# go-compression/raisin

Hardware: AMD Instinct MI355X
Metric: encode+decode MB/s (higher is better)
Workload: dtype u8; 1 GPU; huffman encode+decode, 1024 MiB uniform-random bytes 0x00-0x7F (BASELINE configs[1]), splitmix64 seed 0x5EED0002; algorithm=huffman, bytes_per_gpu=1073741824, chunks=1

## Files before the change

### raisin_amd/csrc/huff_decode.hip

```cpp
#include <chrono>
#include <optional>
#include "codecs.h"
#include "rsn_helpers.h"

namespace rsn {


constexpr int DB = 256;
constexpr int FDB = 256;
constexpr int SW = 8;
constexpr int SBITS = SW * 32;
constexpr int ORG_WORDS = 8;
constexpr int ORG = ORG_WORDS * 32;
constexpr int DATA_WORDS = ORG_WORDS + DB * SW + 8;
constexpr int LUT_BITS_MAX = 11;
constexpr int LUT_WORDS = 1 << LUT_BITS_MAX;
constexpr int OUT_STAGE = DB * 64;
constexpr int OUT_STAGE_RUNE = 40960;
constexpr int CHILD_LDS = 256;
constexpr int LUT2_LDS = 768;
constexpr uint32_t LUT2_GLOBAL_MAX = 1u << 20;
constexpr int SYNC_ROUNDS = 24;
constexpr uint32_t BAD_REL = 0xFFFF;
constexpr uint32_t BAD_POS = 0xFFFFFFFFu;
// ... 219 lines not shown
                }
                const uint32_t er = a.entry_rel[g];
                skip = er == BAD_REL ? e == ~0ull : e == blk_bit0 + er;
            }
            if (__atomic_load_n(a.stuck, __ATOMIC_RELAXED)) skip = 2;
            s_skip = skip;
        }
        __syncthreads();
        if (s_skip == 2) {
            if (live) { a.entry_rel[g] = (uint16_t)BAD_REL; a.exit_rel[g] = (uint16_t)BAD_REL; a.nbyte[g] = 0; }
            if (tid == 0) a.blk_bytes[blk] = 0;
            continue;
        }
        if (s_skip) continue;
        stage_data(a, blk, s_data);
        __syncthreads();

        uint32_t e;
        if (!live) e = BAD_POS;
        else if (g == 0) e = (uint32_t)a.p0 + ORG;
        else if (a.pass == 0 || tid > 0) {
            const long long p0_rel = (long long)a.p0 - (long long)blk_bit0 + ORG;
            if (p0_rel >= (long long)my0) e = (uint32_t)p0_rel;
            else if (a.flat_guess) {
                const unsigned long long d = (unsigned long long)((long long)my0 - p0_rel) + a.min_len - 1;
                e = (uint32_t)(p0_rel + (long long)(d - d % a.min_len));
            } else {
                const uint32_t start = (uint32_t)max(p0_rel, (long long)my0 - a.warm);
                uint32_t q = start;
                (void)advance<ASCII, SHORT, MULTI>(a, s_data, s_lut, lane_r, l2, q, my0, (uint32_t)tid);
                e = q;
            }
        } else {
            const uint32_t xr = a.exit_rel[g - 1];
            e = xr == BAD_REL ? BAD_POS : ORG + xr;
        }
        bool have = false;
        uint32_t x = 0, nb = 0;
        if (live && a.pass > 0 && tid > 0) {
            const uint32_t er = a.entry_rel[g];
            const uint32_t xr = a.exit_rel[g];
            e = er == BAD_REL ? BAD_POS : my0 + er;
            x = xr == BAD_REL ? BAD_POS : lim + xr;
            nb = a.nbyte[g];
            have = true;
        }
        __syncthreads();
        for (int round = 0; round <= DB; round++) {
            if (live && !have) {
                if (e == BAD_POS) { x = BAD_POS; nb = 0; }
                else walk<ASCII, SHORT, MULTI>(a, s_data, s_lut, lane_r, l2, e, lim, (uint32_t)tid + 1u, end_rel, &x, &nb);
                have = true;
            }
            s_exit[tid] = x;
            __syncthreads();
            bool changed = false;
            if (live && tid > 0) {
                const uint32_t en = s_exit[tid - 1];
                if (en != e) { e = en; have = false; changed = true; }
            }
            if (!__syncthreads_or(changed)) break;
            if (round == SYNC_ROUNDS) { if (tid == 0) *a.stuck = 1; break; }
        }
        if (live && !have) { e = BAD_POS; x = BAD_POS; nb = 0; }
        if (live) {
            const uint16_t new_exit = x == BAD_POS ? (uint16_t)BAD_REL : (uint16_t)(x - lim);
            if (a.pass > 0 && tid == DB - 1 && a.exit_rel[g] != new_exit) *a.changed = 1;
            a.entry_rel[g] = e == BAD_POS ? BAD_REL : (uint16_t)(e - my0);
            a.exit_rel[g] = new_exit;
            a.nbyte[g] = (uint16_t)nb;
        }
        unsigned long long sum = live ? nb : 0;
        for (int d = 32; d; d >>= 1) sum += __shfl_down(sum, d);
        if ((tid & 63) == 0) s_part[tid >> 6] = sum;
        __syncthreads();
        if (tid == 0) {
            unsigned long long all = 0;
            for (int k = 0; k < DB / 64; k++) all += s_part[k];
            a.blk_bytes[blk] = all;
        }
    }
}

__global__ __launch_bounds__(256) void k_dec_fix_list(const uint16_t *__restrict__ exit_rel, const uint16_t *__restrict__ entry_rel, uint32_t n_blk,
                                                      uint32_t *__restrict__ list, uint32_t *__restrict__ count) {
    const uint32_t b = blockIdx.x * 256 + threadIdx.x;
    const bool need = b >= 1 && b < n_blk && exit_rel[(size_t)b * DB - 1] != entry_rel[(size_t)b * DB];
    const unsigned long long m = __ballot(need);
    if (!m) return;
    const int lane = threadIdx.x & 63;
    uint32_t base = 0;
    if (lane == 0) base = atomicAdd(count, (uint32_t)__builtin_popcountll(m));
    base = (uint32_t)__builtin_amdgcn_readfirstlane((int)base);
    if (need) list[base + (uint32_t)__builtin_popcountll(m & ((1ull << lane) - 1ull))] = b;
}

constexpr uint32_t PH_CAND = 64;
struct PhaseArgs {
    uint2 *blk_map;
    const uint8_t *true_c;
    uint32_t cand;
};

template <bool ASCII, bool SHORT, bool MULTI>
__global__ __launch_bounds__(DB) void k_dec_phase(DecArgs a, PhaseArgs p, uint32_t n_blk, int mode) {
    __shared__ __attribute__((aligned(1024))) uint32_t s_data[DATA_PHYS];
    __shared__ uint32_t s_lut[LUT_WORDS];
    __shared__ int32_t s_child[SHORT ? 1 : CHILD_LDS];
    __shared__ uint32_t s_lut2[SHORT ? 1 : LUT2_LDS];
    __shared__ uint32_t s_T[64 * PH_CAND];
    const int tid = threadIdx.x;
    const uint32_t lane = tid & 63, wave = tid >> 6;
    const uint32_t lane_r = tid & ((1u << a.rep_log2) - 1);
    stage_lut(a, s_lut);
    if (!SHORT && a.child_n <= (uint32_t)CHILD_LDS) { for (uint32_t i = tid; i < a.child_n; i += DB) s_child[i] = a.child[i]; a.child = s_child; }
    const Lut2 l2{s_lut2, a.lut2_n <= (uint32_t)LUT2_LDS};
    if (!SHORT && l2.in_lds) for (uint32_t i = tid; i < a.lut2_n; i += DB) s_lut2[i] = a.lut2[i];
    for (uint32_t blk = blockIdx.x; blk < n_blk; blk += gridDim.x) {
        const unsigned long long blk_bit0 = (unsigned long long)blk * DB * SBITS;
        const uint32_t L = min((uint32_t)DB, a.n_sub - blk * DB);
        const uint32_t end_rel = (uint32_t)min(a.end - blk_bit0 + ORG, (unsigned long long)(ORG + DB * SBITS + 4096));
        const uint32_t C = p.cand;
        __syncthreads();
        stage_data(a, blk, s_data);
        uint32_t e = mode == 0 ? (uint32_t)tid : (uint32_t)p.true_c[blk];
        if (mode == 2 && e == 0xFF) e = BAD_REL;
        if (blk == 0 && mode == 0 && tid > 0) e = 0x10000u;
        uint32_t bytes = 0;
        const bool follower = mode == 0 ? (uint32_t)tid < C : tid == 0;
        for (uint32_t grp0 = 0; grp0 < L; grp0 += 64) {
            __syncthreads();
            const uint32_t t = grp0 + lane;
            if (t < L) {
                const uint32_t t0 = ORG + t * SBITS, lim = min(t0 + (uint32_t)SBITS, end_rel);
                const uint32_t first = blk == 0 && t == 0 ? (uint32_t)a.p0 : 0u;
                for (uint32_t c0 = wave; c0 < C; c0 += DB / 64) {
                    uint32_t x = BAD_POS, nbs = 0;
                    walk<ASCII, SHORT, MULTI>(a, s_data, s_lut, lane_r, l2, t0 + first + c0, lim, t + 1u, end_rel, &x, &nbs);
                    s_T[lane * PH_CAND + c0] = (x == BAD_POS ? (uint32_t)BAD_REL : x - lim) | nbs << 16;
                }
            }
            __syncthreads();
            if (follower) {
                const uint32_t n_here = min(64u, L - grp0);
                for (uint32_t k = 0; k < n_here; k++) {
                    const uint32_t g = blk * DB + grp0 + k;
                    uint32_t x = BAD_REL, nbs = 0;
                    if (e < C) { const uint32_t v = s_T[k * PH_CAND + e]; x = v & 0xFFFFu; nbs = v >> 16; }
                    else if (e != BAD_REL) e = 0x10000u;
                    if (mode == 2) {
                        a.entry_rel[g] = (uint16_t)(e == BAD_REL || e >= C ? (uint32_t)BAD_REL : (blk == 0 && grp0 + k == 0 ? (uint32_t)a.p0 : e));
                        a.exit_rel[g] = (uint16_t)x; a.nbyte[g] = (uint16_t)nbs;
                    }
                    bytes += nbs;
                    if (e < C || e == BAD_REL) e = x;
                }
            }
        }
        if (follower) {
            if (mode == 0) p.blk_map[(size_t)blk * PH_CAND + tid] = make_uint2(e & 0xFFFFu, e > 0xFFFFu ? 0xFFFFFFFFu : bytes);
            else a.blk_bytes[blk] = bytes;
        }
    }
}

struct Sink {
    uint8_t *wordp; unsigned long long acc; uint32_t cnt, lo;
    __device__ __forceinline__ void start(uint8_t *p) { lo = (uint32_t)((uintptr_t)p & 7); wordp = p - lo; cnt = lo; acc = 0; }
    __device__ __forceinline__ void put(uint32_t b) {
        acc |= (unsigned long long)b << (8 * cnt);
        if (++cnt == 8) {
            if (lo == 0) *reinterpret_cast<unsigned long long *>(wordp) = acc;
            else for (uint32_t k = lo; k < 8; k++) wordp[k] = (uint8_t)(acc >> (8 * k));
            wordp += 8; acc = 0; cnt = 0; lo = 0;
        }
    }
    __device__ __forceinline__ void finish() { for (uint32_t k = lo; k < cnt; k++) wordp[k] = (uint8_t)(acc >> (8 * k)); }
};

template <class Put>
__device__ __forceinline__ void put_rune(uint32_t rune, Put put) {
    if (rune < 0x80) put(rune);
    else if (rune < 0x800) { put(0xC0 | (rune >> 6)); put(0x80 | (rune & 0x3F)); }
    else if (rune < 0x10000) { put(0xE0 | (rune >> 12)); put(0x80 | ((rune >> 6) & 0x3F)); put(0x80 | (rune & 0x3F)); }
    else { put(0xF0 | (rune >> 18)); put(0x80 | ((rune >> 12) & 0x3F)); put(0x80 | ((rune >> 6) & 0x3F)); put(0x80 | (rune & 0x3F)); }
}

template <bool ASCII, bool SHORT, class Put>
__device__ __forceinline__ void emit_walk(const DecArgs &a, const uint32_t *s_data, const uint32_t *s_lut,
                                          uint32_t lane_r, const Lut2 &l2, uint32_t pos, uint32_t lim, Put put) {
    while (pos < lim) {
        const uint32_t r = decode_one<ASCII, SHORT>(a, s_data, s_lut, lane_r, pos, l2);
        if (ASCII) put(r); else put_rune(r, put);
    }
}

#define RSN_EMIT_WORD(p, v) atomicOr((p), (v))
template <bool ASCII, bool SHORT, bool MULTI>
__global__ __launch_bounds__(DB) void k_dec_emit(DecArgs a, uint32_t n_blk) {
    __shared__ __attribute__((aligned(1024))) uint32_t s_data[DATA_PHYS];
    __shared__ uint32_t s_lut[LUT_WORDS];
    constexpr int STAGE = ASCII ? OUT_STAGE : OUT_STAGE_RUNE;
    __shared__ __attribute__((aligned(16))) uint8_t s_out[STAGE + 32];
    __shared__ uint32_t s_wsum[DB / 64];
    __shared__ int32_t s_child[SHORT ? 1 : CHILD_LDS];
    __shared__ uint32_t s_lut2[SHORT ? 1 : LUT2_LDS];
    const int tid = threadIdx.x, lane = tid & 63, wv = tid >> 6;
    const uint32_t lane_r = tid & ((1u << a.rep_log2) - 1);
    const uint32_t my0 = ORG + tid * SBITS;
    stage_lut(a, s_lut);
    if (!SHORT && a.child_n <= (uint32_t)CHILD_LDS) { for (uint32_t i = tid; i < a.child_n; i += DB) s_child[i] = a.child[i]; a.child = s_child; }
    const Lut2 l2{s_lut2, a.lut2_n <= (uint32_t)LUT2_LDS};
    if (!SHORT && l2.in_lds) for (uint32_t i = tid; i < a.lut2_n; i += DB) s_lut2[i] = a.lut2[i];
    if (ASCII) for (int i = tid; i < (STAGE + 32) / 16; i += DB) reinterpret_cast<uint4 *>(s_out)[i] = make_uint4(0, 0, 0, 0);
    for (uint32_t blk = blockIdx.x; blk < n_blk; blk += gridDim.x) {
        const unsigned long long blk_bit0 = (unsigned long long)blk * DB * SBITS;
        const uint32_t g = blk * DB + tid;
        const bool live = g < a.n_sub;
        const uint32_t end_rel = (uint32_t)min(a.end - blk_bit0 + ORG, (unsigned long long)(ORG + DB * SBITS + 4096));
        const uint32_t lim = min(my0 + SBITS, end_rel);
        __syncthreads();
        stage_data(a, blk, s_data);
        const uint32_t nb = live ? a.nbyte[g] : 0;
        const uint32_t er = live ? a.entry_rel[g] : BAD_REL;
        uint32_t incl = nb;
        for (int d = 1; d < 64; d <<= 1) { const uint32_t y = __shfl_up(incl, d); if (lane >= d) incl += y; }
        if (lane == 63) s_wsum[wv] = incl;
        __syncthreads();
        uint32_t wpre = 0, total = 0;
        for (int k = 0; k < DB / 64; k++) { if (k < wv) wpre += s_wsum[k]; total += s_wsum[k]; }
        const uint32_t my_off = wpre + incl - nb;
        if (a.blk_off[blk] + total > a.out_cap) continue;
        uint8_t *dst = a.out + a.blk_off[blk];
        const uint32_t al = (uint32_t)((uintptr_t)dst & 15);
        const bool staged = total + al <= (uint32_t)STAGE;
        if (ASCII && staged) {
            if (live && er != BAD_REL && nb != 0) {
                const uint32_t o0 = al + my_off;
                uint32_t *o = reinterpret_cast<uint32_t *>(s_out) + (o0 >> 2);
                const uint32_t spo = 32u * ((uint32_t)tid + 1u);
                uint32_t cnt = o0 & 3, remaining = nb, pos = my0 + er + spo;
                unsigned long long acc = 0;
                while (remaining) {
                    const uint32_t win = window32_sp(s_data, pos);
                    const uint32_t e = lut_at(a, s_lut, win, lane_r);
                    uint32_t bytes = u_bytes(e);
                    uint32_t take = min(u_n(e), remaining);
                    uint32_t used = u_used(e);
                    if (!SHORT && __ballot((e & 0x80000000u) != 0)) {
                        if (e & 0x80000000u) { uint32_t q = pos - spo; bytes = decode_long(a, s_data, win, e, q, l2); take = 1; used = q + spo - pos; }
                    }
                    acc |= (unsigned long long)bytes << (8 * cnt);
                    cnt += take; remaining -= take; pos += used;
                    if (cnt >= 4) { RSN_EMIT_WORD(o, (uint32_t)acc); o++; acc >>= 32; cnt -= 4; }
                    if (used <= (uint32_t)LUT_BITS_MAX && remaining) {
                        uint32_t e2 = lut_at(a, s_lut, win >> used, lane_r);
                        if (!SHORT) e2 = (int32_t)e2 < 0 ? 0u : e2;
                        {
                            const uint32_t b2 = u_bytes(e2);
                            const uint32_t t2 = min(u_n(e2), remaining);
                            acc |= (unsigned long long)b2 << (8 * cnt);
                            cnt += t2; remaining -= t2; pos += u_used(e2);
                            if (cnt >= 4) { RSN_EMIT_WORD(o, (uint32_t)acc); o++; acc >>= 32; cnt -= 4; }
                        }
                    }
                }
                if (cnt) atomicOr(o, (uint32_t)acc & (0xFFFFFFFFu >> (32 - 8 * cnt)));
            }
        } else if (live && er != BAD_REL && nb != 0) {
            if (staged) {
                uint8_t *o = s_out + al + my_off;
                uint32_t pos = my0 + er;
                emit_walk<ASCII, SHORT>(a, s_data, s_lut, lane_r, l2, pos, lim, [&](uint32_t b) { *o++ = (uint8_t)b; });
            } else {
                Sink sink;
                sink.start(dst + my_off);
                emit_walk<ASCII, SHORT>(a, s_data, s_lut, lane_r, l2, my0 + er, lim, [&](uint32_t b) { sink.put(b); });
                sink.finish();
            }
        }
        if (!staged) continue;
        __syncthreads();
        const uint32_t span = al + total;
        uint8_t *gbase = dst - al;
        for (uint32_t u = tid; u * 16 < span; u += DB) {
            const uint32_t b0 = u * 16;
            if (b0 >= al && b0 + 16 <= span) *reinterpret_cast<uint4 *>(gbase + b0) = *reinterpret_cast<const uint4 *>(s_out + b0);
            else for (uint32_t k = max(b0, al); k < min(b0 + 16, span); k++) gbase[k] = s_out[k];
            if (ASCII) *reinterpret_cast<uint4 *>(s_out + b0) = make_uint4(0, 0, 0, 0);
        }
    }
}

struct FlatArgs {
    const uint8_t *base; size_t nbytes;
    unsigned long long p0;
    unsigned long long n_sym;
    uint8_t *out;
    uint8_t lut[128];
};
constexpr int FLAT_LANE_SYMS = 32;
constexpr int FLAT_SYMS = FDB * FLAT_LANE_SYMS;

template <int L>
__global__ __launch_bounds__(FDB) void k_dec_flat(FlatArgs a) {
    constexpr int WORDS = FDB * L + 2;
    constexpr int RL = 5;
    __shared__ uint32_t s_data[WORDS + WORDS / 32 + 2];
    __shared__ uint32_t s_lut[(1 << L) << RL];
    const int tid = threadIdx.x;
    {
        const uint8_t *lut = (const uint8_t *)__builtin_amdgcn_kernarg_segment_ptr() + offsetof(FlatArgs, lut);
        for (int i = tid; i < ((1 << L) << RL); i += FDB) s_lut[i] = lut[i >> RL];
    }
    const uint32_t n_chunks = (uint32_t)((a.n_sym + FLAT_SYMS - 1) / FLAT_SYMS);
    for (uint32_t chunk = blockIdx.x; chunk < n_chunks; chunk += gridDim.x) {
    const unsigned long long sym0 = (unsigned long long)chunk * FLAT_SYMS;
    const unsigned long long bit0 = a.p0 + sym0 * L;
    const size_t w0 = (size_t)(bit0 >> 5);
    const uint32_t o0 = (uint32_t)(bit0 & 31);
    if ((w0 + WORDS) * 4 <= a.nbytes) {
        const uint32_t *src = reinterpret_cast<const uint32_t *>(a.base) + w0;
        constexpr int PER = (WORDS + FDB - 1) / FDB;
        uint32_t v[PER];
#pragma unroll
        for (int k = 0; k < PER; k++) { const int i = tid + k * FDB; if (i < WORDS) v[k] = ld4<(RSN_NT_MASK & 8) != 0>(src + i); }
#pragma unroll
        for (int k = 0; k < PER; k++) { const int i = tid + k * FDB; if (i < WORDS) s_data[swz(i)] = __builtin_bswap32(v[k]); }
    } else {
        for (int i = tid; i < WORDS; i += FDB) {
            const size_t off = (w0 + i) * 4;
            uint32_t v = 0;
            if (off + 4 <= a.nbytes) v = __builtin_bswap32(*reinterpret_cast<const uint32_t *>(a.base + off));
            else for (int k = 0; k < 4; k++) if (off + k < a.nbytes) v |= (uint32_t)a.base[off + k] << (24 - 8 * k);
            s_data[swz(i)] = v;
        }
    }
    __syncthreads();
    const unsigned long long s_first = sym0 + (unsigned long long)tid * FLAT_LANE_SYMS;
    if (s_first < a.n_sym) {
    const uint32_t lane_r = tid & ((1u << RL) - 1);
    uint32_t w[L + 1], v[L];
#pragma unroll
    for (int j = 0; j <= L; j++) w[j] = s_data[swz(tid * L + j)];
#pragma unroll
    for (int j = 0; j < L; j++) v[j] = (uint32_t)((((unsigned long long)w[j] << 32) | w[j + 1]) >> (32 - o0));
    uint32_t o[8];
#pragma unroll
    for (int k = 0; k < FLAT_LANE_SYMS; k++) {
        constexpr uint32_t mask = (1u << L) - 1;
        const int bp = k * L, wi = bp >> 5, sh = bp & 31;
        uint32_t f;
        if (sh + L <= 32) f = (v[wi] >> (32 - sh - L)) & mask;
        else f = (uint32_t)((((unsigned long long)v[wi] << 32) | v[wi + 1 < L ? wi + 1 : wi]) >> (64 - sh - L)) & mask;
        const uint32_t sym = s_lut[(f << RL) | lane_r];
        if ((k & 3) == 0) o[k >> 2] = sym; else o[k >> 2] |= sym << (8 * (k & 3));
    }
    uint8_t *dst = a.out + s_first;
    if (s_first + FLAT_LANE_SYMS <= a.n_sym) {
        st16<(RSN_NT_MASK & 16) != 0>(reinterpret_cast<uint4 *>(dst), make_uint4(o[0], o[1], o[2], o[3]));
        st16<(RSN_NT_MASK & 16) != 0>(reinterpret_cast<uint4 *>(dst + 16), make_uint4(o[4], o[5], o[6], o[7]));
    } else {
        const uint32_t cnt = (uint32_t)(a.n_sym - s_first);
        for (uint32_t k = 0; k < cnt; k++) dst[k] = (uint8_t)(o[k >> 2] >> (8 * (k & 3)));
    }
    }
    __syncthreads();
    }
}

namespace {

void build_tables(const HuffTree &t, int K, std::vector<uint32_t> &lut, std::vector<int32_t> &child) {
    const uint32_t A = t.n_leaves;
    const size_t n_int = t.freq.size() - A;
    child.assign(2 * std::max<size_t>(n_int, 1), 0);
    for (size_t i = 0; i < n_int; i++) {
        const int32_t id = (int32_t)(A + i);
        const int32_t kids[2] = {t.left[id], t.right[id]};
        for (int b = 0; b < 2; b++)
            child[2 * i + b] = t.is_leaf(kids[b]) ? -(int32_t)(t.rune[kids[b]] + 1) : kids[b] - (int32_t)A;
    }
    lut.assign((size_t)1 << K, 0);
    struct It { int32_t node; uint32_t prefix; int depth; };
    std::vector<It> st;
    st.push_back({t.root, 0, 0});
    while (!st.empty()) {
        const It it = st.back();
        st.pop_back();
        if (t.is_leaf(it.node)) {
            const uint32_t ent = ((uint32_t)it.depth << 24) | t.rune[it.node];
            const uint32_t lo = it.prefix << (K - it.depth);
            for (uint32_t x = 0; x < (1u << (K - it.depth)); x++) lut[lo + x] = ent;
        } else if (it.depth == K) {
            lut[it.prefix] = 0x80000000u | (uint32_t)(it.node - (int32_t)A);
        } else {
            st.push_back({t.right[it.node], (it.prefix << 1) | 1, it.depth + 1});
            st.push_back({t.left[it.node], it.prefix << 1, it.depth + 1});
        }
    }
}

void build_second_level(const std::vector<int32_t> &child, int K, bool byte_alphabet, std::vector<uint32_t> &lut, std::vector<uint32_t> &lut2) {
    lut2.clear();
    const size_t n_int = child.size() / 2;
    std::vector<uint8_t> depth(n_int, 0);
    for (size_t i = 0; i < n_int; i++) {
        unsigned d = 0;
        for (int b = 0; b < 2; b++) { const int32_t k = child[2 * i + b]; d = std::max(d, k < 0 ? 1u : 1u + depth[(size_t)k]); }
        depth[i] = (uint8_t)std::min(d, 255u);
    }
    std::vector<uint32_t> longs;
    for (uint32_t v = 0; v < (1u << K); v++) if (lut[v] & 0x80000000u) longs.push_back(v);
    if (longs.empty()) return;
    auto total = [&](unsigned cap) { uint64_t t = 0; for (uint32_t v : longs) t += 1ull << std::min<unsigned>(depth[lut[v] & 0x3FFFFFFu], cap); return t; };
    unsigned cap = 32u - (unsigned)K;
    if (total(cap) > (uint64_t)LUT2_LDS) {
        const uint64_t budget = byte_alphabet ? (uint64_t)LUT2_LDS : (uint64_t)LUT2_GLOBAL_MAX;
        while (cap > 0 && total(cap) > budget) cap--;
    }
    if (cap == 0) return;
    struct It { int32_t node; uint32_t path; unsigned q; };
    std::vector<It> st;
    for (uint32_t v : longs) {
        const int32_t top = (int32_t)(lut[v] & 0x3FFFFFFu);
        const unsigned sb = std::min<unsigned>(depth[(size_t)top], cap);
        const uint32_t off = (uint32_t)lut2.size();
        lut2.resize(lut2.size() + ((size_t)1 << sb));
        st.push_back({top, 0, 0});
        while (!st.empty()) {
            const It it = st.back();
            st.pop_back();
            if (it.q == sb) { lut2[off + it.path] = 0x80000000u | (uint32_t)it.node; continue; }
            for (int b = 0; b < 2; b++) {
                const int32_t k = child[2 * (size_t)it.node + b];
                const uint32_t path = it.path | ((uint32_t)b << it.q);
                const unsigned q1 = it.q + 1;
                if (k >= 0) { st.push_back({k, path, q1}); continue; }
                const uint32_t ent = ((uint32_t)(K + q1) << 24) | (uint32_t)(-(k + 1));
                for (uint32_t y = 0; y < (1u << (sb - q1)); y++) lut2[off + path + (y << q1)] = ent;
            }
        }
        lut[v] = 0x80000000u | (sb << 26) | off;
    }
}

int rep_for(int K) {
    int r = 0;
    while (r < 5 && ((1 << K) << (r + 1)) <= LUT_WORDS) r++;
    return r;
}

}

int huff_decode_dev(Ctx &c, hipStream_t s, const uint8_t *d_in, size_t n, uint8_t *d_out, size_t out_cap, size_t *out_n, const SliceStream *st) {
    if (((uintptr_t)d_in & 15) || ((uintptr_t)d_out & 15)) return c.fail(RSN_ERR_ARG, "huffman: device buffers must be 16-byte aligned");
    *out_n = 0;
    std::vector<uint8_t> head;
    size_t sep = (size_t)-1;
    for (size_t want = 4096;; want *= 8) {
        const size_t k = std::min(want, n);
        const size_t old = head.size();
        if (k > old) {
            if (st && !st->need_in(k)) return c.fail(RSN_ERR_DEVICE, "huffman: the upload of a sliced call failed");
            void *hpin; int prc = pinned_buf(c, k - old + 64, &hpin); if (prc) return prc;
            RSN_HIP(copy_async(hpin, d_in + old, k - old, hipMemcpyDeviceToHost, s));
            RSN_HIP(hipStreamSynchronize(s));
            head.resize(k);
            memcpy(head.data() + old, hpin, k - old);
        }
        for (size_t i = old ? old - 1 : 0; i + 1 < k; i++) if (head[i] == 0x5C && head[i + 1] == 0x0A) { sep = i; break; }
        if (sep != (size_t)-1 || k == n) break;
    }
    if (sep == (size_t)-1) return c.fail(RSN_ERR_FORMAT, "huffman: no '\\\\\\n' separator (reference: index out of range, huffman.go:264)");
    if (sep + 3 > head.size() && sep + 3 <= n) {
        const size_t old = head.size();
        if (st && !st->need_in(sep + 3)) return c.fail(RSN_ERR_DEVICE, "huffman: the upload of a sliced call failed");
        void *hpin; int prc = pinned_buf(c, 64, &hpin); if (prc) return prc;
        RSN_HIP(copy_async(hpin, d_in + old, sep + 3 - old, hipMemcpyDeviceToHost, s));
        RSN_HIP(hipStreamSynchronize(s));
        head.resize(sep + 3);
        memcpy(head.data() + old, hpin, sep + 3 - old);
    }
    std::vector<HuffSym> syms; std::string msg;
    static const bool host_timing = getenv("RSN_HOST_TIMING") != nullptr;
    auto now = [] { return std::chrono::steady_clock::now(); };
    auto ms = [](std::chrono::steady_clock::time_point a, std::chrono::steady_clock::time_point b) { return std::chrono::duration<double, std::milli>(b - a).count(); };
    const auto t0 = now();
    if (!parse_header(head.data(), sep, syms, msg)) return c.fail(RSN_ERR_FORMAT, "%s", msg.c_str());
    const auto t1 = now();
    const size_t sn = n - sep - 2;
    const unsigned diff = sn ? head[sep + 2] : 0;
    const unsigned long long nbits = sn ? (unsigned long long)(sn - 1) * 8 : 0;
    if (diff > nbits) return c.fail(RSN_ERR_FORMAT, "huffman: pad exceeds the payload (reference: slice bounds out of range, huffman.go:294)");
    const unsigned long long max = nbits - diff;
    if (!d_out) {
        if (syms.empty()) return c.fail(RSN_ERR_FORMAT, "huffman: empty header (reference panics in heap.Pop, huffman.go:102)");
        if (syms.size() == 1) {
            if (max > 0) return c.fail(RSN_ERR_FORMAT, "huffman: single-symbol tree with a non-empty payload (reference recurses without end, huffman.go:139-140)");
            *out_n = 32;
            return c.fail(RSN_ERR_CAPACITY, "huffman: output needs %d bytes by the header's counts", utf8_len(syms[0].rune));
        }
        if (max == 0) return c.fail(RSN_ERR_FORMAT, "huffman: payload ends inside a codeword (reference: index out of range, huffman.go:145)");
        unsigned long long total = 0, expect = 0;
        bool beyond = false;
        for (const HuffSym &sy : syms) {
            if (sy.freq > max - total) { beyond = true; break; }
            total += sy.freq;
            expect += sy.freq * (unsigned long long)utf8_len(sy.rune);
        }
        if (beyond) expect = 4 * max;
        *out_n = round_up((size_t)expect, 16) + 16;
        return c.fail(RSN_ERR_CAPACITY, beyond ? "huffman: output needs at most %llu bytes (the header counts more symbols than the payload holds)"
                                               : "huffman: output needs %llu bytes by the header's counts", expect);
    }
    HuffTree tree; HuffCodes codes;
    if (!build_tree(syms, tree, msg)) return c.fail(RSN_ERR_FORMAT, "%s", msg.c_str());
    const auto t2 = now();
    constexpr int k_env = LUT_BITS_MAX;
    std::vector<uint32_t> lut, lut2; std::vector<int32_t> child;
    const bool prebuilt = tree.n_leaves > 4096;
    std::optional<SideJob> table_builder;
    if (prebuilt) table_builder.emplace([&] { build_tables(tree, k_env, lut, child); build_second_level(child, k_env, false, lut, lut2); });
    const bool codes_ok = assign_codes(tree, codes, msg, false);
    if (prebuilt) table_builder->finish();
    if (!codes_ok) return c.fail(RSN_ERR_LIMIT, "%s", msg.c_str());
    const auto t3 = now();
    if (host_timing) fprintf(stderr, "huffman decode host: header of %zu bytes parsed in %.2f ms, tree %.2f ms, codes %.2f ms, %zu symbols\n", sep, ms(t0, t1), ms(t1, t2), ms(t2, t3), syms.size());

    if (tree.n_leaves == 1) {
        if (max > 0) return c.fail(RSN_ERR_FORMAT, "huffman: single-symbol tree with a non-empty payload (reference recurses without end, huffman.go:139-140)");
        uint8_t u[4];
        const size_t k = (size_t)go_encode_rune(tree.rune[0], u);
        *out_n = k;
        if (!d_out || out_cap < k) { return c.fail(RSN_ERR_CAPACITY, "huffman: output needs %zu bytes", k); }
        RSN_HIP(copy_async(d_out, u, k, hipMemcpyHostToDevice, s));
        RSN_HIP(hipStreamSynchronize(s));
        return RSN_OK;
    }
    if (max == 0) return c.fail(RSN_ERR_FORMAT, "huffman: payload ends inside a codeword (reference: index out of range, huffman.go:145)");

    bool ascii = true;
    for (uint32_t i = 0; i < tree.n_leaves; i++) if (tree.rune[i] >= 0x80) ascii = false;
    const size_t pay = sep + 3;
    const size_t A0 = pay & ~(size_t)15;
    void *p; int rc;

    static const bool no_flat = getenv("RSN_NO_FLAT") != nullptr;
    if (ascii && codes.min_len == codes.max_len && codes.max_len <= 7 && !no_flat) {
        const uint32_t L = codes.max_len;
        if (max % L) return c.fail(RSN_ERR_FORMAT, "huffman: payload ends inside a codeword (reference: index out of range, huffman.go:145)");
        const unsigned long long n_sym = max / L;
        *out_n = (size_t)n_sym;
        if (!d_out || n_sym > out_cap) { *out_n = round_up((size_t)n_sym, 16) + 16; return c.fail(RSN_ERR_CAPACITY, "huffman: output needs %llu bytes, buffer holds %zu", n_sym, out_cap); }
        FlatArgs fa{};
        fa.base = d_in + A0; fa.nbytes = n - A0; fa.p0 = 8ull * (pay - A0) + diff; fa.n_sym = n_sym;
        fa.out = d_out;
        for (uint32_t i = 0; i < tree.n_leaves; i++) fa.lut[codes.code[i]] = (uint8_t)tree.rune[i];
        const unsigned long long per = st ? std::max<unsigned long long>(FLAT_SYMS, (unsigned long long)st->slice_bytes * 8 / L / FLAT_SYMS * FLAT_SYMS) : n_sym;
        const unsigned long long p0_all = fa.p0;
        for (unsigned long long q0 = 0; q0 < n_sym || q0 == 0; q0 += per) {
            const unsigned long long q1 = std::min(n_sym, q0 + per);
            if (st) {
                const size_t upto = std::min(n, A0 + (size_t)((p0_all + q1 * L + 7) / 8) + 4096);
                if (!st->need_in(upto)) return c.fail(RSN_ERR_DEVICE, "huffman: the upload of a sliced call failed");
                fa.nbytes = upto - A0;
            }
            fa.p0 = p0_all + q0 * L; fa.n_sym = q1 - q0; fa.out = d_out + q0;
            const size_t chunks = ceil_div((size_t)(q1 - q0), FLAT_SYMS);
            dim3 grid;
            switch (L) {
#define RSN_FLAT_CASE(LL) case LL:                                                                                \
                rc = persistent_grid(c, reinterpret_cast<const void *>(k_dec_flat<LL>), FDB, chunks, &grid); if (rc) return rc; \
                RSN_LAUNCH("huff_dec_flat", k_dec_flat<LL>, grid, dim3(FDB), 0, s, fa); break;
                RSN_FLAT_CASE(1) RSN_FLAT_CASE(2) RSN_FLAT_CASE(3) RSN_FLAT_CASE(4) RSN_FLAT_CASE(5) RSN_FLAT_CASE(6)
                RSN_FLAT_CASE(7)
#undef RSN_FLAT_CASE
                default: return c.fail(RSN_ERR_LIMIT, "huffman: flat code length %u", L);
            }
            RSN_HIP(hipStreamSynchronize(s));
            if (st && !st->have_out((size_t)q0, (size_t)(q1 - q0))) return c.fail(RSN_ERR_DEVICE, "huffman: the download of a sliced call failed");
            if (q1 >= n_sym) break;
        }
        return RSN_OK;
    }

    const int K = (int)std::min<unsigned>(ascii ? std::max(codes.max_len, 3u * codes.min_len + 2u) : codes.max_len, (unsigned)k_env);
    const bool short_codes = codes.max_len <= (unsigned)K;
    if (!prebuilt) build_tables(tree, K, lut, child);
    const auto t4 = now();
    static const bool no_multi = getenv("RSN_NO_MULTI") != nullptr;
    unsigned long long n_syms_total = 0;
    for (uint32_t i = 0; i < tree.n_leaves; i++) n_syms_total += tree.freq[i];
    const bool multi = ascii && !no_multi && n_syms_total && codes.total_bits * 10 <= n_syms_total * 65;
    if (ascii) {
        const std::vector<uint32_t> plain = lut;
        for (uint32_t v = 0; v < (1u << K); v++) {
            if (plain[v] & 0x80000000u) continue;
            uint32_t used = 0, nsym = 0, syms = 0, len1 = 0;
            while (nsym < 3 && used < (uint32_t)K) {
                int32_t node = tree.root;
                uint32_t q = used;
                while (!tree.is_leaf(node) && q < (uint32_t)K) { node = ((v >> (K - 1 - q)) & 1) ? tree.right[node] : tree.left[node]; q++; }
                if (!tree.is_leaf(node)) break;
                syms |= (tree.rune[node] & 0x7Fu) << (8 * nsym);
                if (nsym == 0) len1 = q;
                used = q; nsym++;
            }
            lut[v] = u_entry(syms, used, nsym, len1);
        }
    }
    if (!prebuilt && !short_codes) build_second_level(child, K, ascii, lut, lut2);
    const auto t5 = now();
    {
        std::vector<uint32_t> t(lut.size());
        for (uint32_t v = 0; v < (1u << K); v++) t[K ? __builtin_bitreverse32(v) >> (32 - K) : 0u] = lut[v];
        lut.swap(t);
    }
    if (host_timing) fprintf(stderr, "huffman decode host: first level + child array %.2f ms, second level %.2f ms (%zu entries), bit-reversal %.2f ms\n", ms(t3, t4), ms(t4, t5), lut2.size(), ms(t5, now()));
    static const bool dbg = getenv("RSN_DEBUG") != nullptr;
    if (dbg) fprintf(stderr, "huffman decode tables: K %d, longest code %u, %zu tree nodes, second level %zu entries (%s)\n", K, codes.max_len, child.size() / 2, lut2.size(), lut2.size() <= (size_t)LUT2_LDS ? "LDS" : "L2");
    rc = dev_buf(c, 5, (lut.size() + child.size() + lut2.size()) * 4 + 64, &p); if (rc) return rc;
    uint32_t *d_lut = (uint32_t *)p;
    int32_t *d_child = (int32_t *)(d_lut + lut.size());
    uint32_t *d_lut2 = (uint32_t *)(d_child + child.size());
    std::vector<uint32_t> packed;
    if (lut.size() + child.size() + lut2.size() <= (64u << 10)) {
        packed.reserve(lut.size() + child.size() + lut2.size());
        packed.insert(packed.end(), lut.begin(), lut.end());
        packed.insert(packed.end(), reinterpret_cast<const uint32_t *>(child.data()), reinterpret_cast<const uint32_t *>(child.data()) + child.size());
        packed.insert(packed.end(), lut2.begin(), lut2.end());
        RSN_HIP(copy_async(d_lut, packed.data(), packed.size() * 4, hipMemcpyHostToDevice, s));
    } else {
        RSN_HIP(copy_async(d_lut, lut.data(), lut.size() * 4, hipMemcpyHostToDevice, s));
        RSN_HIP(copy_async(d_child, child.data(), child.size() * 4, hipMemcpyHostToDevice, s));
        if (!lut2.empty()) RSN_HIP(copy_async(d_lut2, lut2.data(), lut2.size() * 4, hipMemcpyHostToDevice, s));
    }

    void *hp; rc = pinned_buf(c, 64, &hp); if (rc) return rc;
    static const int warm_env = [] { const char *e = getenv("RSN_DEC_WARM"); return e ? atoi(e) : 128; }();
    auto decode_range = [&](const uint8_t *rbase, size_t rnbytes, unsigned long long rp0, unsigned long long rend, unsigned long long rsubs, uint8_t *rout, size_t rcap,
                            size_t *rtotal, uint32_t *rlast) -> int {
    DecArgs a{};
    a.base = rbase; a.nbytes = rnbytes;
    a.p0 = rp0;
    a.end = rend;
    const unsigned long long n_sub64 = rsubs;
    if (n_sub64 > 0xFFFFFF00ull) return c.fail(RSN_ERR_LIMIT, "huffman: payload too large for one call");
    a.n_sub = (uint32_t)n_sub64;
    a.lut = d_lut; a.K = K; a.rep_log2 = rep_for(K); a.child = d_child; a.child_n = (uint32_t)child.size(); a.min_len = codes.min_len;
    a.lut2 = d_lut2; a.lut2_n = (uint32_t)lut2.size();
    a.flat_guess = codes.min_len == codes.max_len;
    a.warm = std::min(std::max(warm_env, 0), ORG - 32);
    const uint32_t n_blk = (uint32_t)ceil_div(a.n_sub, DB);
    rc = dev_buf(c, 6, (size_t)a.n_sub * 6 + 64, &p); if (rc) return rc;
    a.exit_rel = (uint16_t *)p; a.entry_rel = a.exit_rel + a.n_sub; a.nbyte = a.entry_rel + a.n_sub;
    rc = dev_buf(c, 7, ((size_t)n_blk * 2 + 4) * 8 + (size_t)n_blk * 4 + 64, &p); if (rc) return rc;
    a.blk_bytes = (unsigned long long *)p;
    unsigned long long *d_blk_off = a.blk_bytes + n_blk;
    unsigned long long *d_total = d_blk_off + n_blk;
    int *d_changed = (int *)(d_total + 1);
    int *d_stuck = (int *)(d_total + 2);
    a.stuck = d_stuck;
    uint32_t *d_fix_count = (uint32_t *)(d_changed + 1);
    uint32_t *d_fix_list = (uint32_t *)(d_total + 4);
    a.changed = d_changed;

    constexpr uint32_t grid_env = 256u * 8u * 2u;
    const uint32_t grid_p = std::min<uint32_t>(n_blk, grid_env);
    auto launch_sync = [&]() -> int {
        const char *nm = a.pass == 0 ? "huff_dec_sync" : a.pass == 1 ? "huff_dec_sync_fix" : "huff_dec_sync_verify";
        if (multi && short_codes) RSN_LAUNCH(nm, (k_dec_sync<true, true, true>), dim3(grid_p), dim3(DB), 0, s, a, n_blk);
        else if (multi) RSN_LAUNCH(nm, (k_dec_sync<true, false, true>), dim3(grid_p), dim3(DB), 0, s, a, n_blk);
        else if (ascii && short_codes) RSN_LAUNCH(nm, (k_dec_sync<true, true, false>), dim3(grid_p), dim3(DB), 0, s, a, n_blk);
        else if (ascii) RSN_LAUNCH(nm, (k_dec_sync<true, false, false>), dim3(grid_p), dim3(DB), 0, s, a, n_blk);
        else if (short_codes) RSN_LAUNCH(nm, (k_dec_sync<false, true, false>), dim3(grid_p), dim3(DB), 0, s, a, n_blk);
        else RSN_LAUNCH(nm, (k_dec_sync<false, false, false>), dim3(grid_p), dim3(DB), 0, s, a, n_blk);
        return RSN_OK;
    };
    a.blk_off = d_blk_off; a.out = rout; a.out_cap = rcap;
    struct Tail { unsigned long long total; uint16_t last_exit; int changed; int stuck; };
    Tail *ht = (Tail *)hp;
    auto launch_emit = [&]() -> int {
        if (ascii && short_codes) RSN_LAUNCH("huff_dec_emit", (k_dec_emit<true, true, false>), dim3(grid_p), dim3(DB), 0, s, a, n_blk);
        else if (ascii) RSN_LAUNCH("huff_dec_emit", (k_dec_emit<true, false, false>), dim3(grid_p), dim3(DB), 0, s, a, n_blk);
        else if (short_codes) RSN_LAUNCH("huff_dec_emit", (k_dec_emit<false, true, false>), dim3(grid_p), dim3(DB), 0, s, a, n_blk);
        else RSN_LAUNCH("huff_dec_emit", (k_dec_emit<false, false, false>), dim3(grid_p), dim3(DB), 0, s, a, n_blk);
        return RSN_OK;
    };
    auto offsets_and_bytes = [&]() -> int {
        int rc2 = scan_u64(c, s, "huff_dec_scan", a.blk_bytes, d_blk_off, n_blk, d_total); if (rc2) return rc2;
        rc2 = launch_emit(); if (rc2) return rc2;
        RSN_HIP(copy_async(&ht->total, d_total, 8, hipMemcpyDeviceToHost, s));
        RSN_HIP(copy_async(&ht->last_exit, a.exit_rel + (a.n_sub - 1), 2, hipMemcpyDeviceToHost, s));
        RSN_HIP(copy_async(&ht->stuck, d_stuck, 4, hipMemcpyDeviceToHost, s));
        return RSN_OK;
    };
    auto phase_solve = [&]() -> int {
        static const bool dbg2 = getenv("RSN_DEBUG") != nullptr;
        const auto ph_t0 = std::chrono::steady_clock::now();
        auto ph_ms = [&]() { return std::chrono::duration<double, std::milli>(std::chrono::steady_clock::now() - ph_t0).count(); };
        const size_t nbk = n_blk;
        void *pp2; int r2 = dev_buf(c, 34, nbk * (PH_CAND * 8 + 1) + 256, &pp2); if (r2) return r2;
        PhaseArgs ph{};
        ph.blk_map = (uint2 *)pp2;
        uint8_t *d_true = (uint8_t *)(ph.blk_map + PH_CAND * nbk);
        ph.true_c = d_true;
        ph.cand = std::min<uint32_t>(PH_CAND, std::max<uint32_t>(codes.max_len, 1));
        auto launch_phase = [&](int mode) -> int {
            const char *nm = mode == 0 ? "huff_dec_phase" : "huff_dec_phase_write";
            if (multi && short_codes) RSN_LAUNCH(nm, (k_dec_phase<true, true, true>), dim3(grid_p), dim3(DB), 0, s, a, ph, n_blk, mode);
            else if (multi) RSN_LAUNCH(nm, (k_dec_phase<true, false, true>), dim3(grid_p), dim3(DB), 0, s, a, ph, n_blk, mode);
            else if (ascii && short_codes) RSN_LAUNCH(nm, (k_dec_phase<true, true, false>), dim3(grid_p), dim3(DB), 0, s, a, ph, n_blk, mode);
            else if (ascii) RSN_LAUNCH(nm, (k_dec_phase<true, false, false>), dim3(grid_p), dim3(DB), 0, s, a, ph, n_blk, mode);
            else if (short_codes) RSN_LAUNCH(nm, (k_dec_phase<false, true, false>), dim3(grid_p), dim3(DB), 0, s, a, ph, n_blk, mode);
            else RSN_LAUNCH(nm, (k_dec_phase<false, false, false>), dim3(grid_p), dim3(DB), 0, s, a, ph, n_blk, mode);
            return RSN_OK;
        };
        void *hq; r2 = pinned_buf(c, 64 + nbk * PH_CAND * 8, &hq); if (r2) return r2;
        hp = hq;
        ht = (Tail *)hq;
        ht->changed = 1;
        uint2 *hmap = (uint2 *)((uint8_t *)hq + 64);
        r2 = launch_phase(0); if (r2) return r2;
        RSN_HIP(copy_async(hmap, ph.blk_map, nbk * PH_CAND * 8, hipMemcpyDeviceToHost, s));
        RSN_HIP(hipStreamSynchronize(s));
        if (dbg2) fprintf(stderr, "huffman decode, phases: +%.3f ms: every entry of every lane walked, the blocks' maps on the host\n", ph_ms());
        std::vector<uint8_t> tc(nbk, 0xFF);
        uint32_t e = 0;
        for (size_t b = 0; b < nbk; b++) {
            if (b + 16 < nbk) for (uint32_t k = 0; k < ph.cand; k += 8) __builtin_prefetch(&hmap[(b + 16) * PH_CAND + k]);
            if (e == BAD_REL) break;
            if (e >= ph.cand) { if (dbg2) fprintf(stderr, "huffman decode, phases: block %zu is entered at bit %u\n", b, e); return 1; }
            const uint2 m = hmap[b * PH_CAND + e];
            if (m.y == 0xFFFFFFFFu) { if (dbg2) fprintf(stderr, "huffman decode, phases: block %zu has no path from bit %u\n", b, e); return 1; }
            tc[b] = (uint8_t)e;
            e = m.x;
        }
        if (dbg2) fprintf(stderr, "huffman decode, phases: +%.3f ms: the blocks chained\n", ph_ms());
        RSN_HIP(copy_async(d_true, tc.data(), nbk, hipMemcpyHostToDevice, s));
        r2 = launch_phase(2); if (r2) return r2;
        RSN_HIP(hipStreamSynchronize(s));
        if (dbg2) fprintf(stderr, "huffman decode, phases: +%.3f ms: the true path written\n", ph_ms());
        if (dbg2) fprintf(stderr, "huffman decode: settled by every entry of every lane (%u blocks, %u entries a lane)\n", n_blk, ph.cand);
        return RSN_OK;
    };
    a.pass = 0;
    RSN_HIP(hipMemsetAsync(d_stuck, 0, 4, s));
    rc = launch_sync(); if (rc) return rc;
    ht->changed = 0; ht->stuck = 0;
    if (n_blk > 1) {
        a.pass = 1;
        RSN_HIP(hipMemsetAsync(d_changed, 0, 8, s));
        RSN_LAUNCH("huff_dec_fix_list", k_dec_fix_list, dim3((uint32_t)ceil_div(n_blk, 256)), dim3(256), 0, s, (const uint16_t *)a.exit_rel, (const uint16_t *)a.entry_rel, n_blk, d_fix_list, d_fix_count);
        a.fix_list = d_fix_list; a.fix_count = d_fix_count;
        rc = launch_sync(); if (rc) return rc;
        RSN_HIP(copy_async(&ht->changed, d_changed, 4, hipMemcpyDeviceToHost, s));
    }
    rc = offsets_and_bytes(); if (rc) return rc;
    RSN_HIP(hipStreamSynchronize(s));
    if (ht->stuck) {
        const int prc = phase_solve();
        if (prc < 0) return prc;
        if (prc != RSN_OK) return c.fail(RSN_ERR_DEVICE, "huffman: synchronisation did not converge");
        rc = offsets_and_bytes(); if (rc) return rc;
        RSN_HIP(hipStreamSynchronize(s));
    } else if (ht->changed) {
        static const bool dbg_p = getenv("RSN_DEBUG") != nullptr;
        for (uint32_t pass = 2; ht->changed; pass++) {
            if (dbg_p) fprintf(stderr, "huffman decode: pass %u, still moving\n", pass);
// ... 66 lines not shown
```

### raisin_amd/csrc/rsn_common.h

```cpp
#pragma once

#include <hip/hip_runtime.h>

#include <cstdarg>
#include <cstdint>
#include <cstdio>
#include <cstdlib>
#include <cstring>
#include <algorithm>
#include <atomic>
#include <mutex>
#include <string>
#include <vector>

#include "../../include/rsn.h"

namespace rsn {

struct ProfSlot {
    std::string name;
    uint64_t launches = 0;
    double total_ms = 0;
    std::vector<std::pair<hipEvent_t, hipEvent_t>> pending;
};

struct Ctx {
    int device = 0;
    bool device_chosen = false;
    bool inited = false;
    hipStream_t own_stream = nullptr;
    std::string err;
    bool prof = false;
    std::vector<ProfSlot> slots;
    std::vector<hipEvent_t> free_events;

    struct Buf { void *p = nullptr; size_t cap = 0; unsigned long long gen = 0; };
    enum { N_BUFS = 43 };
    Buf bufs[N_BUFS];
    void *pinned = nullptr; size_t pinned_cap = 0;
    bool lz_runs = false;
    size_t gate_held = 0;

    ~Ctx();

    int fail(int code, const char *fmt, ...) {
        char tmp[512];
        va_list ap; va_start(ap, fmt); vsnprintf(tmp, sizeof tmp, fmt, ap); va_end(ap);
        err = tmp;
        return code;
    }
};

Ctx &ctx();
int ctx_init(Ctx &c);
int dev_buf(Ctx &c, int slot, size_t bytes, void **out);
int pinned_buf(Ctx &c, size_t bytes, void **out);
size_t scratch_admit(Ctx &c, size_t need);
void scratch_release(Ctx &c, size_t held, unsigned long long slots);
void scratch_forget(Ctx &c, size_t bytes);
unsigned long long scratch_queued(int device);
void prof_collect(Ctx &c);
int func_dyn_lds(Ctx &c, const void *fn, size_t bytes);

#define RSN_HIP(call)                                                                              \
    do {                                                                                           \
        hipError_t e__ = (call);                                                                   \
        if (e__ != hipSuccess)                                                                     \
            return c.fail(RSN_ERR_DEVICE, "%s failed: %s (%s:%d)", #call, hipGetErrorString(e__),  \
                          __FILE__, __LINE__);                                                     \
    } while (0)

inline int persistent_grid(Ctx &c, const void *fn, int block, size_t work, dim3 *grid) {
    struct Entry { const void *fn; int device, block; uint32_t blocks; };
    static std::mutex mu;
    static std::vector<Entry> *seen = new std::vector<Entry>();
    uint32_t blocks = 0;
    {
        std::lock_guard<std::mutex> lk(mu);
        for (const Entry &e : *seen)
            if (e.fn == fn && e.device == c.device && e.block == block) { blocks = e.blocks; break; }
        if (!blocks) {
            int per_cu = 0, cus = 0;
            RSN_HIP(hipOccupancyMaxActiveBlocksPerMultiprocessor(&per_cu, fn, block, 0));
            RSN_HIP(hipDeviceGetAttribute(&cus, hipDeviceAttributeMultiprocessorCount, c.device));
            if (per_cu < 1 || cus < 1) return c.fail(RSN_ERR_DEVICE, "occupancy query: %d blocks of %d threads a CU on %d CUs", per_cu, block, cus);
            blocks = (uint32_t)per_cu * (uint32_t)cus;
            seen->push_back({fn, c.device, block, blocks});
        }
    }
    *grid = dim3((uint32_t)std::min<size_t>(work, blocks));
    return RSN_OK;
}

struct CopyCount { std::atomic<int> on{0}; std::atomic<unsigned long long> h2d{0}, d2h{0}; };
inline CopyCount g_copy_count;
inline hipError_t copy_async(void *dst, const void *src, size_t bytes, hipMemcpyKind kind, hipStream_t s) {
    if (g_copy_count.on.load(std::memory_order_relaxed)) {
        if (kind == hipMemcpyHostToDevice) g_copy_count.h2d.fetch_add(bytes, std::memory_order_relaxed);
        else if (kind == hipMemcpyDeviceToHost) g_copy_count.d2h.fetch_add(bytes, std::memory_order_relaxed);
    }
    return hipMemcpyAsync(dst, src, bytes, kind, s);
}

struct ProfScope {
    Ctx &c; hipStream_t s; int slot = -1; hipEvent_t a = nullptr, b = nullptr;
    ProfScope(Ctx &c_, hipStream_t s_, const char *name) : c(c_), s(s_) {
        if (!c.prof) return;
        for (size_t i = 0; i < c.slots.size(); i++) if (c.slots[i].name == name) slot = (int)i;
        if (slot < 0) { c.slots.emplace_back(); c.slots.back().name = name; slot = (int)c.slots.size() - 1; }
        auto get = [&]() { hipEvent_t e = nullptr; if (!c.free_events.empty()) { e = c.free_events.back(); c.free_events.pop_back(); } else (void)hipEventCreate(&e); return e; };
        a = get(); b = get();
        (void)hipEventRecord(a, s);
    }
    ~ProfScope() {
        if (slot < 0) return;
        (void)hipEventRecord(b, s);
        c.slots[slot].pending.emplace_back(a, b);
    }
};

#define RSN_LAUNCH(name, kernel, grid, block, shmem, stream, ...)                                  \
    do {                                                                                           \
        {                                                                                          \
            rsn::ProfScope ps__(c, stream, name);                                                  \
            hipLaunchKernelGGL(kernel, grid, block, shmem, stream, __VA_ARGS__);                   \
        }                                                                                          \
        RSN_HIP(hipGetLastError());                                                                \
    } while (0)

#ifndef RSN_NT_MASK
#define RSN_NT_MASK 1
#endif
#ifdef __HIPCC__
typedef uint32_t rsn_u32x4 __attribute__((ext_vector_type(4)));
typedef uint32_t rsn_u32x4_a4 __attribute__((ext_vector_type(4), aligned(4)));
template <bool NT> __device__ __forceinline__ uint4 ld16(const uint4 *p) {
    if constexpr (NT) { const rsn_u32x4 v = __builtin_nontemporal_load(reinterpret_cast<const rsn_u32x4 *>(p)); return make_uint4(v.x, v.y, v.z, v.w); }
    else return *p;
}
template <bool NT> __device__ __forceinline__ uint32_t ld4(const uint32_t *p) {
    if constexpr (NT) return __builtin_nontemporal_load(p);
    else return *p;
}
template <bool NT> __device__ __forceinline__ void st16(uint4 *p, const uint4 &v) {
    if constexpr (NT) { rsn_u32x4 x = {v.x, v.y, v.z, v.w}; __builtin_nontemporal_store(x, reinterpret_cast<rsn_u32x4 *>(p)); }
    else *p = v;
}
template <bool NT> __device__ __forceinline__ void st16_a4(uint32_t *p, uint32_t a, uint32_t b, uint32_t c_, uint32_t d) {
    rsn_u32x4_a4 x = {a, b, c_, d};
    if constexpr (NT) __builtin_nontemporal_store(x, reinterpret_cast<rsn_u32x4_a4 *>(p));
    else *reinterpret_cast<rsn_u32x4_a4 *>(p) = x;
}
#endif

static inline size_t ceil_div(size_t a, size_t b) { return (a + b - 1) / b; }
static inline size_t round_up(size_t a, size_t b) { return ceil_div(a, b) * b; }

}
```

Before: 1.012 million MB/s.

## Vectorize flat decoder loads, coalesce output via DPP lane swap, post header via kernel

The flat Huffman decoder now loads its compressed window with 16-byte loads and uses a new per-width LDS swizzle. Lanes are regrouped so that adjacent lane pairs exchange halves through a DPP swap, letting each wave write contiguous 16-byte segments instead of strided 32-byte pieces. The initial 4 KiB header fetch is replaced by a small kernel that writes into pinned host memory and sets a flag, which the host spins on instead of doing a memcpy plus stream synchronize. This adds bank-layout complexity and a host polling path with a timeout fallback.

```diff
diff --git a/raisin_amd/csrc/huff_decode.hip b/raisin_amd/csrc/huff_decode.hip
--- a/raisin_amd/csrc/huff_decode.hip
+++ b/raisin_amd/csrc/huff_decode.hip
@@ -545,17 +545,24 @@
 constexpr int FLAT_LANE_SYMS = 32;
 constexpr int FLAT_SYMS = FDB * FLAT_LANE_SYMS;
 
+template <int L> __device__ __forceinline__ constexpr uint32_t fswz(uint32_t i) {
+    if constexpr (L & 1) return i ^ (((i >> 5) & 1u) << 4);
+    else if constexpr (L == 4) return i + (i >> 2) + (i >> 7) * 16;
+    else return i + (i >> 6) * 15 + (i >> 7) * 2;
+}
+
 template <int L>
 __global__ __launch_bounds__(FDB) void k_dec_flat(FlatArgs a) {
     constexpr int WORDS = FDB * L + 2;
     constexpr int RL = 5;
-    __shared__ uint32_t s_data[WORDS + WORDS / 32 + 2];
+    __shared__ __attribute__((aligned(16))) uint32_t s_data[((L & 1) ? (uint32_t)WORDS + 16 : fswz<L>(WORDS)) + 4];
     __shared__ uint32_t s_lut[(1 << L) << RL];
-    const int tid = threadIdx.x;
+    const int tid = threadIdx.x, lane = tid & 63;
     {
         const uint8_t *lut = (const uint8_t *)__builtin_amdgcn_kernarg_segment_ptr() + offsetof(FlatArgs, lut);
         for (int i = tid; i < ((1 << L) << RL); i += FDB) s_lut[i] = lut[i >> RL];
     }
+    const uint32_t grp = (uint32_t)(tid & ~63) | ((uint32_t)(lane & 1) << 5) | (uint32_t)(lane >> 1);
     const uint32_t n_chunks = (uint32_t)((a.n_sym + FLAT_SYMS - 1) / FLAT_SYMS);
     for (uint32_t chunk = blockIdx.x; chunk < n_chunks; chunk += gridDim.x) {
     const unsigned long long sym0 = (unsigned long long)chunk * FLAT_SYMS;
@@ -564,28 +571,40 @@
     const uint32_t o0 = (uint32_t)(bit0 & 31);
     if ((w0 + WORDS) * 4 <= a.nbytes) {
         const uint32_t *src = reinterpret_cast<const uint32_t *>(a.base) + w0;
-        constexpr int PER = (WORDS + FDB - 1) / FDB;
-        uint32_t v[PER];
+        constexpr int NQ = WORDS / 4, PER = (NQ + FDB - 1) / FDB;
+        uint4 v[PER];
+        uint32_t tail = 0;
 #pragma unroll
-        for (int k = 0; k < PER; k++) { const int i = tid + k * FDB; if (i < WORDS) v[k] = ld4<(RSN_NT_MASK & 8) != 0>(src + i); }
+        for (int k = 0; k < PER; k++) { const int q = tid + k * FDB; if (q < NQ) v[k] = ld16_a4<(RSN_NT_MASK & 8) != 0>(src + 4 * q); }
+        if (tid < WORDS - 4 * NQ) tail = ld4<(RSN_NT_MASK & 8) != 0>(src + 4 * NQ + tid);
 #pragma unroll
-        for (int k = 0; k < PER; k++) { const int i = tid + k * FDB; if (i < WORDS) s_data[swz(i)] = __builtin_bswap32(v[k]); }
+        for (int k = 0; k < PER; k++) {
+            const int q = tid + k * FDB;
+            if (q < NQ) {
+                uint32_t *d = s_data + fswz<L>(4 * q);
+                const uint32_t x = __builtin_bswap32(v[k].x), y = __builtin_bswap32(v[k].y), z = __builtin_bswap32(v[k].z), w = __builtin_bswap32(v[k].w);
+                if constexpr (L & 1) *reinterpret_cast<uint4 *>(d) = make_uint4(x, y, z, w);
+                else { d[0] = x; d[1] = y; d[2] = z; d[3] = w; }
+            }
+        }
+        if (tid < WORDS - 4 * NQ) s_data[fswz<L>(4 * NQ + tid)] = __builtin_bswap32(tail);
     } else {
         for (int i = tid; i < WORDS; i += FDB) {
             const size_t off = (w0 + i) * 4;
             uint32_t v = 0;
             if (off + 4 <= a.nbytes) v = __builtin_bswap32(*reinterpret_cast<const uint32_t *>(a.base + off));
             else for (int k = 0; k < 4; k++) if (off + k < a.nbytes) v |= (uint32_t)a.base[off + k] << (24 - 8 * k);
-            s_data[swz(i)] = v;
+            s_data[fswz<L>(i)] = v;
         }
     }
     __syncthreads();
-    const unsigned long long s_first = sym0 + (unsigned long long)tid * FLAT_LANE_SYMS;
-    if (s_first < a.n_sym) {
+    const bool whole = sym0 + FLAT_SYMS <= a.n_sym;
+    const unsigned long long s_first = sym0 + (unsigned long long)grp * FLAT_LANE_SYMS;
+    if (whole || s_first < a.n_sym) {
     const uint32_t lane_r = tid & ((1u << RL) - 1);
     uint32_t w[L + 1], v[L];
 #pragma unroll
-    for (int j = 0; j <= L; j++) w[j] = s_data[swz(tid * L + j)];
+    for (int j = 0; j <= L; j++) w[j] = s_data[fswz<L>(grp * L + j)];
 #pragma unroll
     for (int j = 0; j < L; j++) v[j] = (uint32_t)((((unsigned long long)w[j] << 32) | w[j + 1]) >> (32 - o0));
     uint32_t o[8];
@@ -599,17 +618,38 @@
         const uint32_t sym = s_lut[(f << RL) | lane_r];
         if ((k & 3) == 0) o[k >> 2] = sym; else o[k >> 2] |= sym << (8 * (k & 3));
     }
-    uint8_t *dst = a.out + s_first;
-    if (s_first + FLAT_LANE_SYMS <= a.n_sym) {
-        st16<(RSN_NT_MASK & 16) != 0>(reinterpret_cast<uint4 *>(dst), make_uint4(o[0], o[1], o[2], o[3]));
-        st16<(RSN_NT_MASK & 16) != 0>(reinterpret_cast<uint4 *>(dst + 16), make_uint4(o[4], o[5], o[6], o[7]));
+    if (whole) {
+        const bool odd = lane & 1;
+        uint32_t r[4];
+#pragma unroll
+        for (int q = 0; q < 4; q++) r[q] = (uint32_t)__builtin_amdgcn_update_dpp(0, (int)(odd ? o[q] : o[4 + q]), 0xB1, 0xF, 0xF, false);
+        uint8_t *dst = a.out + sym0 + (size_t)(tid & ~63) * FLAT_LANE_SYMS + (size_t)lane * 16;
+        st16<(RSN_NT_MASK & 16) != 0>(reinterpret_cast<uint4 *>(dst), odd ? make_uint4(r[0], r[1], r[2], r[3]) : make_uint4(o[0], o[1], o[2], o[3]));
+        st16<(RSN_NT_MASK & 16) != 0>(reinterpret_cast<uint4 *>(dst + 1024), odd ? make_uint4(o[4], o[5], o[6], o[7]) : make_uint4(r[0], r[1], r[2], r[3]));
     } else {
-        const uint32_t cnt = (uint32_t)(a.n_sym - s_first);
-        for (uint32_t k = 0; k < cnt; k++) dst[k] = (uint8_t)(o[k >> 2] >> (8 * (k & 3)));
+        uint8_t *dst = a.out + s_first;
+        if (s_first + FLAT_LANE_SYMS <= a.n_sym) {
+            st16<(RSN_NT_MASK & 16) != 0>(reinterpret_cast<uint4 *>(dst), make_uint4(o[0], o[1], o[2], o[3]));
+            st16<(RSN_NT_MASK & 16) != 0>(reinterpret_cast<uint4 *>(dst + 16), make_uint4(o[4], o[5], o[6], o[7]));
+        } else {
+            const uint32_t cnt = (uint32_t)(a.n_sym - s_first);
+            for (uint32_t k = 0; k < cnt; k++) dst[k] = (uint8_t)(o[k >> 2] >> (8 * (k & 3)));
+        }
     }
     }
     __syncthreads();
     }
+}
+
+constexpr size_t HEAD_FIRST = 4096;
+__global__ __launch_bounds__(256) void k_head_post(const uint8_t *__restrict__ in, uint32_t k, uint8_t *__restrict__ host, uint32_t *flag, uint32_t seq) {
+    for (uint32_t b = threadIdx.x * 16; b < k; b += 256 * 16) {
+        if (b + 16 <= k) *reinterpret_cast<uint4 *>(host + b) = *reinterpret_cast<const uint4 *>(in + b);
+        else for (uint32_t i = b; i < k; i++) host[i] = in[i];
+    }
+    __threadfence_system();
+    __syncthreads();
+    if (threadIdx.x == 0) __hip_atomic_store(flag, seq, __ATOMIC_RELEASE, __HIP_MEMORY_SCOPE_SYSTEM);
 }
 
 namespace {
@@ -701,14 +741,23 @@
     *out_n = 0;
     std::vector<uint8_t> head;
     size_t sep = (size_t)-1;
-    for (size_t want = 4096;; want *= 8) {
+    for (size_t want = HEAD_FIRST;; want *= 8) {
         const size_t k = std::min(want, n);
         const size_t old = head.size();
         if (k > old) {
             if (st && !st->need_in(k)) return c.fail(RSN_ERR_DEVICE, "huffman: the upload of a sliced call failed");
             void *hpin; int prc = pinned_buf(c, k - old + 64, &hpin); if (prc) return prc;
-            RSN_HIP(copy_async(hpin, d_in + old, k - old, hipMemcpyDeviceToHost, s));
-            RSN_HIP(hipStreamSynchronize(s));
+            if (old == 0 && k <= HEAD_FIRST) {
+                uint32_t *flag = reinterpret_cast<uint32_t *>((uint8_t *)hpin + round_up(k, 16));
+                const uint32_t seq = next_post_seq(c);
+                *(volatile uint32_t *)flag = 0;
+                hipLaunchKernelGGL(k_head_post, dim3(1), dim3(256), 0, s, d_in, (uint32_t)k, (uint8_t *)hpin, flag, seq);
+                RSN_HIP(hipGetLastError());
+                prc = wait_posted(c, s, flag, seq, "the header fetch"); if (prc) return prc;
+            } else {
+                RSN_HIP(copy_async(hpin, d_in + old, k - old, hipMemcpyDeviceToHost, s));
+                RSN_HIP(hipStreamSynchronize(s));
+            }
             head.resize(k);
             memcpy(head.data() + old, hpin, k - old);
         }
diff --git a/raisin_amd/csrc/rsn_common.h b/raisin_amd/csrc/rsn_common.h
--- a/raisin_amd/csrc/rsn_common.h
+++ b/raisin_amd/csrc/rsn_common.h
@@ -9,6 +9,7 @@
 #include <cstring>
 #include <algorithm>
 #include <atomic>
+#include <chrono>
 #include <mutex>
 #include <string>
 #include <vector>
@@ -40,6 +41,7 @@
     void *pinned = nullptr; size_t pinned_cap = 0;
     bool lz_runs = false;
     size_t gate_held = 0;
+    uint32_t post_seq = 0;
 
     ~Ctx();
 
@@ -102,6 +104,22 @@
     return hipMemcpyAsync(dst, src, bytes, kind, s);
 }
 
+inline uint32_t next_post_seq(Ctx &c) { if (++c.post_seq == 0) ++c.post_seq; return c.post_seq; }
+inline int wait_posted(Ctx &c, hipStream_t s, const uint32_t *flag, uint32_t seq, const char *who) {
+    const volatile uint32_t *vf = flag;
+    const auto t0 = std::chrono::steady_clock::now();
+    for (uint32_t spins = 1;; spins++) {
+        if (*vf == seq) { std::atomic_thread_fence(std::memory_order_acquire); return RSN_OK; }
+        if ((spins & 1023) == 0 && std::chrono::steady_clock::now() - t0 > std::chrono::milliseconds(20)) {
+            RSN_HIP(hipStreamSynchronize(s));
+            if (*vf != seq) return c.fail(RSN_ERR_DEVICE, "huffman: %s finished without its answer", who);
+            std::atomic_thread_fence(std::memory_order_acquire);
+            return RSN_OK;
+        }
+        __builtin_ia32_pause();
+    }
+}
+
 struct ProfScope {
     Ctx &c; hipStream_t s; int slot = -1; hipEvent_t a = nullptr, b = nullptr;
     ProfScope(Ctx &c_, hipStream_t s_, const char *name) : c(c_), s(s_) {
@@ -138,6 +156,12 @@
     if constexpr (NT) { const rsn_u32x4 v = __builtin_nontemporal_load(reinterpret_cast<const rsn_u32x4 *>(p)); return make_uint4(v.x, v.y, v.z, v.w); }
     else return *p;
 }
+template <bool NT> __device__ __forceinline__ uint4 ld16_a4(const uint32_t *p) {
+    rsn_u32x4_a4 v;
+    if constexpr (NT) v = __builtin_nontemporal_load(reinterpret_cast<const rsn_u32x4_a4 *>(p));
+    else v = *reinterpret_cast<const rsn_u32x4_a4 *>(p);
+    return make_uint4(v.x, v.y, v.z, v.w);
+}
 template <bool NT> __device__ __forceinline__ uint32_t ld4(const uint32_t *p) {
     if constexpr (NT) return __builtin_nontemporal_load(p);
     else return *p;
```

New measurement: 1.012 million MB/s (median of 2 runs). No clear change (+0.1%).
